# 0xPolygonZero/proof-protocol-decoder

Measured on AMD Instinct MI355X. Metric: txn-proofs/sec (whole node), 256-txn synthetic block, higher is better.
Workload: dtype u64 (Goldilocks field)

## Files before the change

__graft_entry__.py:

```python
import os
import subprocess
import sys

ROOT = os.path.dirname(os.path.abspath(__file__))
if ROOT not in sys.path:
    sys.path.insert(0, ROOT)


def build():
    csrc = os.path.join(ROOT, "proof_protocol_decoder_amd", "csrc")
    subprocess.run(["make", "-C", csrc, "-j8"], check=True)
    subprocess.run(["make", "-C", os.path.join(ROOT, "oracle"), "liboracle.so"], check=True)
    tools = os.path.join(ROOT, "tools")
    subprocess.run(["/opt/rocm/bin/hipcc", "--offload-arch=gfx950", "-O3", "-std=c++17", "-Wno-unused-value", "-o",
                    os.path.join(tools, "microbench"), os.path.join(tools, "microbench.hip")], check=True)
    subprocess.run(["/opt/rocm/bin/hipcc", "--offload-arch=gfx950", "-O2", "-Wno-unused-value", "-o",
                    os.path.join(tools, "wait_probe"), os.path.join(tools, "wait_probe.hip")], check=True)
    subprocess.run(["/opt/rocm/bin/hipcc", "--offload-arch=gfx950", "-O3", "-Wno-unused-value", "-o",
                    os.path.join(tools, "issue_rate"), os.path.join(tools, "issue_rate.hip")], check=True)
    subprocess.run(["/opt/rocm/bin/hipcc", "--offload-arch=gfx950", "-O3", "-Wno-unused-value", "-o",
                    os.path.join(tools, "mfma_probe"), os.path.join(tools, "mfma_probe.hip")], check=True)
    subprocess.run(["/opt/rocm/bin/hipcc", "--offload-arch=gfx950", "-O3", "-std=c++17", "-Wno-unused-value", "-I", csrc,
                    "-mllvm", "-amdgpu-mfma-vgpr-form=1", "-o", os.path.join(tools, "perm_latency"),
                    os.path.join(tools, "perm_latency.hip")], check=True)
    import proof_protocol_decoder_amd as pkg
    pkg.lib()
    return None


def smoke():
    import numpy as np
    import torch
    assert torch.cuda.is_available(), "smoke() needs a GPU"
    import proof_protocol_decoder_amd as pkg
    from proof_protocol_decoder_amd import proof_gen as pg
    from oracle import pyoracle
    sys.path.insert(0, os.path.join(ROOT, "tests"))
    from pg_common import LOG_N, SMALL_PLONK as SMALL, WIDTH, ir_words
    pkg.lib()
    b = pg.ProverStateBuilder()
    for t, name in enumerate(pg.TABLES):
        getattr(b, "set_%s_circuit_size" % name)(range(SMALL["table_log_lo"][t], SMALL["table_log_hi"][t]))
    b.set(**{k: v for k, v in SMALL.items() if not k.startswith("table_")}, n_workers=1, arena_bytes=256 << 20)
    st = b.build()
    try:
        t0 = pg.generate_txn_proof(st, pg.TxnProofGenIR(7, 0, 100, 121, (1, 2, 3, 4), 0x5EED0001, LOG_N, WIDTH))
        t1 = pg.generate_txn_proof(st, pg.TxnProofGenIR(7, 1, 121, 150, t0.p_vals.state_root_after, 0x5EED0002,
                                                        LOG_N, WIDTH))
        agg = pg.generate_agg_proof(st, t0, t1)
        blk = pg.generate_block_proof(st, None, agg)
        pg.VerifierState.from_prover_state(st).verify(blk)
        pyoracle.build()
        ost = pyoracle.PgState(**SMALL)
        want = ost.txn(ir_words(7, 0, 0x5EED0001))
        got = np.frombuffer(t0.intern, dtype=np.uint64)
        assert got.shape == want.shape and (got == want).all(), "txn proof differs from the oracle"
        assert ost.verify(np.frombuffer(blk.intern, dtype=np.uint64)) == 0, "oracle verifier rejected the block proof"
    finally:
        st.close()
    print("smoke ok: txn proof == oracle (%d bytes), block proof verified by both verifiers" % len(t0.intern))
    return None


if __name__ == "__main__":
    build()
    if len(sys.argv) > 1 and sys.argv[1] == "smoke":
        smoke()
```

proof_protocol_decoder_amd/csrc/mx_arith.cuh:

```cuda
#pragma once
#include "gl.hpp"

namespace mxa {

typedef int v4i __attribute__((ext_vector_type(4)));

template <int N>
__device__ __forceinline__ void reduce_rows(const uint64_t (&L)[N], const uint64_t (&H)[N], uint64_t (&out)[N]) {
  uint32_t l0[N], l1[N], h0[N], h1[N];
  uint64_t T[N];
  gl::cc::mask c1[N], b[N];
#pragma unroll
  for (int i = 0; i < N; i++) {
    T[i] = L[i]; h0[i] = (uint32_t)H[i]; h1[i] = (uint32_t)(H[i] >> 32);
  }
  gl::cc::mad_eps_cv(T, h1);
#pragma unroll
  for (int i = 0; i < N; i++) { l0[i] = (uint32_t)T[i]; l1[i] = (uint32_t)(T[i] >> 32); }
  gl::cc::add_co(l1, c1, h0);
  gl::cc::subb0_co(l0, b, c1);
#pragma unroll
  for (int i = 0; i < N; i++) c1[i] &= ~b[i];
  gl::cc::addc0_cv(l1, c1);
#pragma unroll
  for (int i = 0; i < N; i++) out[i] = gl::cc::mk64(l0[i], l1[i]);
}


__device__ __forceinline__ uint64_t planes(const v4i& d) {
  const uint32_t e = (uint32_t)d[0] + ((uint32_t)d[1] << 8), f = (uint32_t)d[2] + ((uint32_t)d[3] << 8);
  uint64_t r;
  asm("v_mad_u64_u32 %0, vcc, %1, %2, %3" : "=v"(r) : "v"(f), "s"(65536u), "v"((uint64_t)e) : "vcc");
  return r;
}

}
```

proof_protocol_decoder_amd/csrc/poseidon_mx.cuh:

```cuda
#pragma once
#include "poseidon.cuh"
#include "poseidon_group.hpp"

namespace poseidon {
namespace mx {

using mxa::v4i;

constexpr int CIN_PER_ROUND = 4 * 24;
constexpr int CIN_WORDS = 30 * CIN_PER_ROUND;

__device__ __forceinline__ uint32_t mds_entry(uint32_t i, uint32_t k) {
  constexpr uint32_t C[12] = {17, 15, 41, 16, 2, 28, 13, 13, 39, 18, 34, 20};
  const uint32_t d = (k + 12 - i) % 12;
  uint32_t v = 0;
#pragma unroll
  for (int j = 0; j < 12; j++) v = d == (uint32_t)j ? C[j] : v;
  return v + ((i | k) == 0 ? 8u : 0u);
}

struct CinTable {
  uint32_t v[CIN_WORDS];
};
constexpr CinTable make_cin_table() {
  constexpr uint64_t rc[360] = {
#include "poseidon_rc.inc"
  };
  CinTable t{};
  for (int i = 0; i < CIN_WORDS; i++) {
    const int rnd = i / CIN_PER_ROUND, rem = i % CIN_PER_ROUND, ib = rem / 24, idx = rem % 24;
    const int g = idx >> 3, h = (idx >> 2) & 1, reg = idx & 3, wo = ib + 4 * g;
    uint32_t v = 128u * (256u + (wo == 0 ? 8u : 0u));
    if (rnd < 29) v += (uint32_t)(rc[(rnd + 1) * 12 + wo] >> (8 * (4 * h + reg))) & 0xFFu;
    t.v[i] = v;
  }
  return t;
}
static __device__ const CinTable CIN_TABLE __attribute__((aligned(16))) = make_cin_table();

__device__ __forceinline__ void build_cin(uint32_t* __restrict__ cin) {
  const uint4* src = (const uint4*)CIN_TABLE.v;
  uint4* dst = (uint4*)cin;
  for (uint32_t i = threadIdx.x; i < (uint32_t)CIN_WORDS / 4; i += blockDim.x) dst[i] = src[i];
}

struct Ctx {
  v4i A[3];
  uint32_t kb;
  const uint32_t* cin;
};
__device__ __forceinline__ Ctx make_ctx(const uint32_t* cin_lds) {
  Ctx c;
  const uint32_t lane = threadIdx.x & 63, r = lane & 15;
  c.kb = lane >> 4;
#pragma unroll
  for (int g = 0; g < 3; g++) {
#pragma unroll
    for (int a = 0; a < 3; a++) c.A[g][a] = (int)(mds_entry((r >> 2) + 4 * g, c.kb + 4 * a) << (8 * (r & 3)));
    c.A[g][3] = 0;
  }
  c.cin = cin_lds + c.kb * 24;
  return c;
}

using mxa::planes;

template <int NS>
__device__ __forceinline__ void mds(uint64_t (&e)[NS][3], const Ctx& c, int rnd) {
  const v4i* cr = (const v4i*)(c.cin + rnd * CIN_PER_ROUND);
  v4i cin[6];
#pragma unroll
  for (int t = 0; t < 6; t++) cin[t] = cr[t];
#pragma unroll
  for (int m = 0; m < NS; m++) {
    v4i blo, bhi;
#pragma unroll
    for (int a = 0; a < 3; a++) {
      blo[a] = (int)((uint32_t)e[m][a] ^ 0x80808080u);
      bhi[a] = (int)((uint32_t)(e[m][a] >> 32) ^ 0x80808080u);
    }
    blo[3] = 0;
    bhi[3] = 0;
    uint64_t L[3], H[3];
#pragma unroll
    for (int g = 0; g < 3; g++) {
      const v4i dl = __builtin_amdgcn_mfma_i32_16x16x64_i8(c.A[g], blo, cin[2 * g], 0, 0, 0);
      const v4i dh = __builtin_amdgcn_mfma_i32_16x16x64_i8(c.A[g], bhi, cin[2 * g + 1], 0, 0, 0);
      L[g] = planes(dl);
      H[g] = planes(dh);
    }
    reduce_rows<3>(L, H, e[m]);
  }
}

template <int NS>
__device__ __forceinline__ void sbox_word0(uint64_t (&e)[NS][3], const Ctx& c) {
  if constexpr (NS == 4) {
    uint32_t l0 = (uint32_t)e[0][0], l1 = (uint32_t)e[1][0], l2 = (uint32_t)e[2][0], l3 = (uint32_t)e[3][0];
    uint32_t h0 = (uint32_t)(e[0][0] >> 32), h1 = (uint32_t)(e[1][0] >> 32), h2 = (uint32_t)(e[2][0] >> 32),
             h3 = (uint32_t)(e[3][0] >> 32);
    asm("s_nop 1\n\t"
        "v_permlane16_swap_b32 %0, %1\n\tv_permlane16_swap_b32 %2, %3\n\t"
        "v_permlane16_swap_b32 %4, %5\n\tv_permlane16_swap_b32 %6, %7\n\t"
        "s_nop 0\n\t"
        "v_permlane32_swap_b32 %0, %2\n\tv_permlane32_swap_b32 %4, %6\n\ts_nop 1"
        : "+v"(l0), "+v"(l1), "+v"(l2), "+v"(l3), "+v"(h0), "+v"(h1), "+v"(h2), "+v"(h3));
    const uint64_t y = sbox(gl::cc::mk64(l0, h0));
    l0 = (uint32_t)y;
    h0 = (uint32_t)(y >> 32);
    asm("s_nop 1\n\t"
        "v_permlane32_swap_b32 %0, %2\n\tv_permlane32_swap_b32 %4, %6\n\t"
        "s_nop 1\n\t"
        "v_permlane16_swap_b32 %0, %1\n\tv_permlane16_swap_b32 %2, %3\n\t"
        "v_permlane16_swap_b32 %4, %5\n\tv_permlane16_swap_b32 %6, %7\n\ts_nop 1"
        : "+v"(l0), "+v"(l1), "+v"(l2), "+v"(l3), "+v"(h0), "+v"(h1), "+v"(h2), "+v"(h3));
    e[0][0] = gl::cc::mk64(l0, h0);
    e[1][0] = gl::cc::mk64(l1, h1);
    e[2][0] = gl::cc::mk64(l2, h2);
    e[3][0] = gl::cc::mk64(l3, h3);
  } else if constexpr (NS == 2) {
    uint32_t l0 = (uint32_t)e[0][0], l1 = (uint32_t)e[1][0], h0 = (uint32_t)(e[0][0] >> 32), h1 = (uint32_t)(e[1][0] >> 32);
    asm("s_nop 1\n\tv_permlane16_swap_b32 %0, %1\n\tv_permlane16_swap_b32 %2, %3\n\ts_nop 1"
        : "+v"(l0), "+v"(l1), "+v"(h0), "+v"(h1));
    const uint64_t y = sbox(gl::cc::mk64(l0, h0));
    const bool word0 = c.kb < 2;
    l0 = word0 ? (uint32_t)y : l0;
    h0 = word0 ? (uint32_t)(y >> 32) : h0;
    asm("s_nop 1\n\tv_permlane16_swap_b32 %0, %1\n\tv_permlane16_swap_b32 %2, %3\n\ts_nop 1"
        : "+v"(l0), "+v"(l1), "+v"(h0), "+v"(h1));
    e[0][0] = gl::cc::mk64(l0, h0);
    e[1][0] = gl::cc::mk64(l1, h1);
  } else {
    static_assert(NS == 1, "1, 2 or 4 sets per wave");
    const uint64_t y = sbox(e[0][0]);
    e[0][0] = c.kb == 0 ? y : e[0][0];
  }
}

template <int NS>
__device__ __forceinline__ void sbox_full(uint64_t (&e)[NS][3]) {
#pragma unroll
  for (int m = 0; m < NS; m++) {
    sbox_n<3>(e[m]);
    __builtin_amdgcn_sched_barrier(0);
  }
}

namespace grp {
constexpr int K = 8;
constexpr poseidon::group::Layout LAY = poseidon::group::layout(K);
constexpr int SHORT_K = 6;
constexpr int OPS_WORDS = LAY.n_ops * 256;
constexpr int C_WORDS = poseidon::group::CFORM_WORDS + poseidon::group::CMAIN_WORDS;
constexpr int MDS_A_WORDS = 3 * 256;
template <int NG> constexpr int TABLE_WORDS = OPS_WORDS + NG * C_WORDS + MDS_A_WORDS;
template <int NG> constexpr int IMAGE_WORDS = TABLE_WORDS<NG> + (NG == 3 ? 18 * 256 : 0);

template <int NG>
__device__ __forceinline__ void load_tables(uint32_t* __restrict__ lds, const uint32_t* __restrict__ glob) {
  const uint4* src = (const uint4*)glob;
  uint4* dst = (uint4*)lds;
  for (uint32_t i = threadIdx.x; i < (uint32_t)TABLE_WORDS<NG> / 4; i += blockDim.x) dst[i] = src[i];
}

template <int F>
__device__ __forceinline__ void gather(uint32_t (&l)[4], uint32_t (&h)[4]) {
  if constexpr ((F & 1) == 0)
    asm("s_nop 1\n\t"
        "v_permlane16_swap_b32 %0, %1\n\tv_permlane16_swap_b32 %2, %3\n\t"
        "v_permlane16_swap_b32 %4, %5\n\tv_permlane16_swap_b32 %6, %7\n\t"
        "s_nop 0\n\t"
        "v_permlane32_swap_b32 %0, %2\n\tv_permlane32_swap_b32 %4, %6\n\ts_nop 1"
        : "+v"(l[0]), "+v"(l[1]), "+v"(l[2]), "+v"(l[3]), "+v"(h[0]), "+v"(h[1]), "+v"(h[2]), "+v"(h[3]));
  else
    asm("s_nop 1\n\t"
        "v_permlane16_swap_b32 %0, %1\n\tv_permlane16_swap_b32 %2, %3\n\t"
        "v_permlane16_swap_b32 %4, %5\n\tv_permlane16_swap_b32 %6, %7\n\t"
        "s_nop 0\n\t"
        "v_permlane32_swap_b32 %1, %3\n\tv_permlane32_swap_b32 %5, %7\n\ts_nop 1"
        : "+v"(l[0]), "+v"(l[1]), "+v"(l[2]), "+v"(l[3]), "+v"(h[0]), "+v"(h[1]), "+v"(h[2]), "+v"(h[3]));
}
template <int F>
__device__ __forceinline__ void scatter(uint32_t (&l)[4], uint32_t (&h)[4]) {
  if constexpr ((F & 1) == 0)
    asm("s_nop 1\n\t"
        "v_permlane32_swap_b32 %0, %2\n\tv_permlane32_swap_b32 %4, %6\n\t"
        "s_nop 1\n\t"
        "v_permlane16_swap_b32 %0, %1\n\tv_permlane16_swap_b32 %2, %3\n\t"
        "v_permlane16_swap_b32 %4, %5\n\tv_permlane16_swap_b32 %6, %7\n\ts_nop 1"
        : "+v"(l[0]), "+v"(l[1]), "+v"(l[2]), "+v"(l[3]), "+v"(h[0]), "+v"(h[1]), "+v"(h[2]), "+v"(h[3]));
  else
    asm("s_nop 1\n\t"
        "v_permlane32_swap_b32 %1, %3\n\tv_permlane32_swap_b32 %5, %7\n\t"
        "s_nop 1\n\t"
        "v_permlane16_swap_b32 %0, %1\n\tv_permlane16_swap_b32 %2, %3\n\t"
        "v_permlane16_swap_b32 %4, %5\n\tv_permlane16_swap_b32 %6, %7\n\ts_nop 1"
        : "+v"(l[0]), "+v"(l[1]), "+v"(l[2]), "+v"(l[3]), "+v"(h[0]), "+v"(h[1]), "+v"(h[2]), "+v"(h[3]));
}

struct State {
  v4i blo[4], bhi[4], bsig[4];
  v4i acc[4][2];
};

template <int J>
__device__ __forceinline__ void step(State& s, uint64_t (&e)[4][3], const v4i* ops, const int* cform, uint32_t lane,
                                     bool full = true) {
  constexpr int P = J / 4, F = J % 4;
  const uint32_t kb = lane >> 4;
  if constexpr (F == 0) {
    constexpr int nw = LAY.w_per_half[P];
#pragma unroll
    for (int half = 0; half < 2; half++) {
      const v4i c0 = ((const v4i*)(cform + (P * 2 + half) * 16))[kb];
      const v4i a_lo = ops[(LAY.w_base[P] + half * nw) * 64 + lane], a_hi = ops[(LAY.w_base[P] + half * nw + 1) * 64 + lane];
#pragma unroll
      for (int m = 0; m < 4; m++) {
        s.acc[m][half] = __builtin_amdgcn_mfma_i32_16x16x64_i8(a_lo, s.blo[m], c0, 0, 0, 0);
        s.acc[m][half] = __builtin_amdgcn_mfma_i32_16x16x64_i8(a_hi, s.bhi[m], s.acc[m][half], 0, 0, 0);
      }
      if constexpr (P > 0) {
        const v4i a_sg = ops[(LAY.w_base[P] + half * nw + 2) * 64 + lane];
#pragma unroll
        for (int m = 0; m < 4; m++) s.acc[m][half] = __builtin_amdgcn_mfma_i32_16x16x64_i8(a_sg, s.bsig[m], s.acc[m][half], 0, 0, 0);
      }
    }
  }
  uint32_t l[4], h[4];
  if constexpr (J == 0) {
#pragma unroll
    for (int m = 0; m < 4; m++) { l[m] = (uint32_t)e[m][0]; h[m] = (uint32_t)(e[m][0] >> 32); }
  } else {
    uint64_t L[4], H[4], x[4];
#pragma unroll
    for (int m = 0; m < 4; m++) { L[m] = planes(s.acc[m][0]); H[m] = planes(s.acc[m][1]); }
    reduce_rows<4>(L, H, x);
#pragma unroll
    for (int m = 0; m < 4; m++) { l[m] = (uint32_t)x[m]; h[m] = (uint32_t)(x[m] >> 32); }
  }
  gather<F>(l, h);
  const uint64_t y = sbox(gl::cc::mk64(l[F], h[F])) ^ 0x8080808080808080ULL;
  l[F] = (uint32_t)y;
  h[F] = (uint32_t)(y >> 32);
  scatter<F>(l, h);
#pragma unroll
  for (int m = 0; m < 4; m++) {
    s.bsig[m][2 * (J / 4)] = __builtin_amdgcn_update_dpp(s.bsig[m][2 * (J / 4)], (int)l[m], 0xE4, 1 << F, 0xF, false);
    s.bsig[m][2 * (J / 4) + 1] = __builtin_amdgcn_update_dpp(s.bsig[m][2 * (J / 4) + 1], (int)h[m], 0xE4, 1 << F, 0xF, false);
  }
  if constexpr (J >= LAY.d_first[P] && J < LAY.d_first[P] + LAY.d_count[P]) {
    if (J == SHORT_K - 1 && !full) return;
#pragma unroll
    for (int half = 0; half < 2; half++) {
      const v4i a = ops[(LAY.d_base[P] + 2 * (J - LAY.d_first[P]) + half) * 64 + lane];
#pragma unroll
      for (int m = 0; m < 4; m++) s.acc[m][half] = __builtin_amdgcn_mfma_i32_16x16x64_i8(a, s.bsig[m], s.acc[m][half], 0, 0, 0);
    }
  }
}

template <int NG>
__device__ __forceinline__ void partial_group(uint64_t (&e)[4][3], const uint32_t* tab, const uint32_t* __restrict__ gtab, int grp) {
  const uint32_t lane = threadIdx.x & 63, kb = lane >> 4;
  const bool full = NG == 2 || grp < 2;
  const v4i* ops = (const v4i*)tab;
  const int* cform = (const int*)(tab + OPS_WORDS + grp * C_WORDS);
  const int* cmain = cform + poseidon::group::CFORM_WORDS;
  State s;
#pragma unroll
  for (int m = 0; m < 4; m++) {
#pragma unroll
    for (int a = 0; a < 3; a++) {
      s.blo[m][a] = (int)((uint32_t)e[m][a] ^ 0x80808080u);
      s.bhi[m][a] = (int)((uint32_t)(e[m][a] >> 32) ^ 0x80808080u);
    }
    s.blo[m][3] = 0;
    s.bhi[m][3] = 0;
    s.bsig[m] = v4i{0, 0, 0, 0};
  }
  step<0>(s, e, ops, cform, lane);
  step<1>(s, e, ops, cform, lane);
  step<2>(s, e, ops, cform, lane);
  step<3>(s, e, ops, cform, lane);
  step<4>(s, e, ops, cform, lane);
  step<5>(s, e, ops, cform, lane, full);
  if (full) {
    step<6>(s, e, ops, cform, lane);
    step<7>(s, e, ops, cform, lane);
  }
  const v4i* lops = ops + LAY.main_base * 64 + lane;
  const v4i* gops = (const v4i*)(gtab + TABLE_WORDS<NG>) + lane;
#pragma unroll
  for (int g = 0; g < 3; g++) {
    v4i d[4][2], A[2][3];
    if (full) {
#pragma unroll
      for (int h = 0; h < 2; h++)
#pragma unroll
        for (int c = 0; c < 3; c++) A[h][c] = lops[((g * 2 + h) * 3 + c) * 64];
    } else {
#pragma unroll
      for (int h = 0; h < 2; h++)
#pragma unroll
        for (int c = 0; c < 3; c++) A[h][c] = gops[((g * 2 + h) * 3 + c) * 64];
    }
#pragma unroll
    for (int h = 0; h < 2; h++) {
      const v4i c0 = ((const v4i*)(cmain + (g * 2 + h) * 16))[kb];
#pragma unroll
      for (int m = 0; m < 4; m++) {
        d[m][h] = __builtin_amdgcn_mfma_i32_16x16x64_i8(A[h][0], s.blo[m], c0, 0, 0, 0);
        d[m][h] = __builtin_amdgcn_mfma_i32_16x16x64_i8(A[h][1], s.bhi[m], d[m][h], 0, 0, 0);
        d[m][h] = __builtin_amdgcn_mfma_i32_16x16x64_i8(A[h][2], s.bsig[m], d[m][h], 0, 0, 0);
      }
    }
    uint64_t L[4], H[4], x[4];
#pragma unroll
    for (int m = 0; m < 4; m++) { L[m] = planes(d[m][0]); H[m] = planes(d[m][1]); }
    reduce_rows<4>(L, H, x);
#pragma unroll
    for (int m = 0; m < 4; m++) e[m][g] = x[m];
  }
}
}

template <int NG> constexpr int CIN_GROUPED_ROUNDS = NG == 3 ? 8 : 14;
template <int NG> constexpr int CIN_GROUPED_WORDS = CIN_GROUPED_ROUNDS<NG> * CIN_PER_ROUND;
template <int NG> __device__ __forceinline__ int cin_slot(int rnd) { return rnd < 4 ? rnd : rnd - (30 - CIN_GROUPED_ROUNDS<NG>); }
template <int NG>
__device__ __forceinline__ void build_cin_grouped(uint32_t* __restrict__ cin) {
  const uint4* src = (const uint4*)CIN_TABLE.v;
  uint4* dst = (uint4*)cin;
  for (uint32_t i = threadIdx.x; i < (uint32_t)CIN_GROUPED_WORDS<NG> / 4; i += blockDim.x)
    dst[i] = src[i < 4 * CIN_PER_ROUND / 4 ? i : i + (30 - CIN_GROUPED_ROUNDS<NG>) * CIN_PER_ROUND / 4];
}

template <int NG>
__device__ __forceinline__ void mds4_lds(uint64_t (&e)[4][3], const Ctx& c, int rnd, const uint32_t* tab) {
  const v4i* cr = (const v4i*)(c.cin + cin_slot<NG>(rnd) * CIN_PER_ROUND);
  const v4i* am = (const v4i*)(tab + grp::OPS_WORDS + NG * grp::C_WORDS) + (threadIdx.x & 63);
#pragma unroll
  for (int m = 0; m < 4; m++) {
    v4i blo, bhi;
#pragma unroll
    for (int a = 0; a < 3; a++) {
      blo[a] = (int)((uint32_t)e[m][a] ^ 0x80808080u);
      bhi[a] = (int)((uint32_t)(e[m][a] >> 32) ^ 0x80808080u);
    }
    blo[3] = 0;
    bhi[3] = 0;
    uint64_t L[3], H[3];
#pragma unroll
    for (int g = 0; g < 3; g++) {
      const v4i A = am[g * 64];
      const v4i dl = __builtin_amdgcn_mfma_i32_16x16x64_i8(A, blo, cr[2 * g], 0, 0, 0);
      const v4i dh = __builtin_amdgcn_mfma_i32_16x16x64_i8(A, bhi, cr[2 * g + 1], 0, 0, 0);
      L[g] = planes(dl);
      H[g] = planes(dh);
    }
    reduce_rows<3>(L, H, e[m]);
  }
}

template <int NG>
__device__ __forceinline__ void permute_grouped(uint64_t (&e)[4][3], const Ctx& c, const uint32_t* tab,
                                                const uint32_t* __restrict__ gtab) {
#pragma unroll
  for (int a = 0; a < 3; a++) {
    const uint64_t k = RC[c.kb + 4 * a];
#pragma unroll
    for (int m = 0; m < 4; m++) e[m][a] = gl::add(e[m][a], k);
  }
  int rnd = 0;
#pragma unroll 1
  for (int k = 0; k < 4; k++, rnd++) {
    sbox_full<4>(e);
    mds4_lds<NG>(e, c, rnd, tab);
  }
#pragma unroll 1
  for (int g = 0; g < NG; g++) grp::partial_group<NG>(e, tab, gtab, g);
  rnd = NG == 3 ? 26 : 20;
  if constexpr (NG == 2) {
#pragma unroll 1
    for (; rnd < 26; rnd++) {
      sbox_word0<4>(e, c);
      mds4_lds<NG>(e, c, rnd, tab);
    }
  }
#pragma unroll 1
  for (int k = 0; k < 4; k++, rnd++) {
    sbox_full<4>(e);
    mds4_lds<NG>(e, c, rnd, tab);
  }
}

template <int NS>
__device__ __forceinline__ void permute(uint64_t (&e)[NS][3], const Ctx& c) {
#pragma unroll
  for (int a = 0; a < 3; a++) {
    const uint64_t k = RC[c.kb + 4 * a];
#pragma unroll
    for (int m = 0; m < NS; m++) e[m][a] = gl::add(e[m][a], k);
  }
  int rnd = 0;
#pragma unroll 1
  for (int k = 0; k < 4; k++, rnd++) {
    sbox_full<NS>(e);
    mds<NS>(e, c, rnd);
  }
#pragma unroll 1
  for (int k = 0; k < 22; k++, rnd++) {
    sbox_word0<NS>(e, c);
    mds<NS>(e, c, rnd);
  }
#pragma unroll 1
  for (int k = 0; k < 4; k++, rnd++) {
    sbox_full<NS>(e);
    mds<NS>(e, c, rnd);
  }
}

}
}
```

Measured before the change: 33.55.

## Replace permlane gather/scatter in grouped Poseidon partial rounds with rotated operand addressing

```diff
diff --git a/__graft_entry__.py b/__graft_entry__.py
--- a/__graft_entry__.py
+++ b/__graft_entry__.py
@@ -23,6 +23,10 @@
     subprocess.run(["/opt/rocm/bin/hipcc", "--offload-arch=gfx950", "-O3", "-std=c++17", "-Wno-unused-value", "-I", csrc,
                     "-mllvm", "-amdgpu-mfma-vgpr-form=1", "-o", os.path.join(tools, "perm_latency"),
                     os.path.join(tools, "perm_latency.hip")], check=True)
+    for out, flags in (("mfma_coexec_probe", ["-mllvm", "-amdgpu-mfma-vgpr-form=1"]),
+                       ("mfma_coexec_probe_agpr", ['-DMFMA_FORM="AGPRs"'])):
+        subprocess.run(["/opt/rocm/bin/hipcc", "--offload-arch=gfx950", "-O3", "-std=c++17", "-Wno-unused-value", "-I", csrc]
+                       + flags + ["-o", os.path.join(tools, out), os.path.join(tools, "mfma_coexec_probe.hip")], check=True)
     import proof_protocol_decoder_amd as pkg
     pkg.lib()
     return None
diff --git a/proof_protocol_decoder_amd/csrc/mx_arith.cuh b/proof_protocol_decoder_amd/csrc/mx_arith.cuh
--- a/proof_protocol_decoder_amd/csrc/mx_arith.cuh
+++ b/proof_protocol_decoder_amd/csrc/mx_arith.cuh
@@ -26,6 +26,14 @@
   for (int i = 0; i < N; i++) out[i] = gl::cc::mk64(l0[i], l1[i]);
 }
 
+__device__ __forceinline__ uint64_t reduce_row(uint64_t L, uint64_t H) {
+  uint64_t T;
+  asm("v_mad_u64_u32 %0, vcc, %1, -1, %2" : "=v"(T) : "v"((uint32_t)(H >> 32)), "v"(L) : "vcc");
+  gl::cc::mask c1, b, unused;
+  const uint32_t l1 = gl::cc::add_co((uint32_t)(T >> 32), (uint32_t)H, c1);
+  const uint32_t l0 = gl::cc::subb0_co((uint32_t)T, c1, b);
+  return gl::cc::mk64(l0, gl::cc::addc0_co(l1, c1 & ~b, unused));
+}
 
 __device__ __forceinline__ uint64_t planes(const v4i& d) {
   const uint32_t e = (uint32_t)d[0] + ((uint32_t)d[1] << 8), f = (uint32_t)d[2] + ((uint32_t)d[3] << 8);
diff --git a/proof_protocol_decoder_amd/csrc/poseidon_mx.cuh b/proof_protocol_decoder_amd/csrc/poseidon_mx.cuh
--- a/proof_protocol_decoder_amd/csrc/poseidon_mx.cuh
+++ b/proof_protocol_decoder_amd/csrc/poseidon_mx.cuh
@@ -163,66 +163,83 @@
   for (uint32_t i = threadIdx.x; i < (uint32_t)TABLE_WORDS<NG> / 4; i += blockDim.x) dst[i] = src[i];
 }
 
-template <int F>
-__device__ __forceinline__ void gather(uint32_t (&l)[4], uint32_t (&h)[4]) {
-  if constexpr ((F & 1) == 0)
-    asm("s_nop 1\n\t"
-        "v_permlane16_swap_b32 %0, %1\n\tv_permlane16_swap_b32 %2, %3\n\t"
-        "v_permlane16_swap_b32 %4, %5\n\tv_permlane16_swap_b32 %6, %7\n\t"
-        "s_nop 0\n\t"
-        "v_permlane32_swap_b32 %0, %2\n\tv_permlane32_swap_b32 %4, %6\n\ts_nop 1"
-        : "+v"(l[0]), "+v"(l[1]), "+v"(l[2]), "+v"(l[3]), "+v"(h[0]), "+v"(h[1]), "+v"(h[2]), "+v"(h[3]));
-  else
-    asm("s_nop 1\n\t"
-        "v_permlane16_swap_b32 %0, %1\n\tv_permlane16_swap_b32 %2, %3\n\t"
-        "v_permlane16_swap_b32 %4, %5\n\tv_permlane16_swap_b32 %6, %7\n\t"
-        "s_nop 0\n\t"
-        "v_permlane32_swap_b32 %1, %3\n\tv_permlane32_swap_b32 %5, %7\n\ts_nop 1"
-        : "+v"(l[0]), "+v"(l[1]), "+v"(l[2]), "+v"(l[3]), "+v"(h[0]), "+v"(h[1]), "+v"(h[2]), "+v"(h[3]));
-}
-template <int F>
-__device__ __forceinline__ void scatter(uint32_t (&l)[4], uint32_t (&h)[4]) {
-  if constexpr ((F & 1) == 0)
-    asm("s_nop 1\n\t"
-        "v_permlane32_swap_b32 %0, %2\n\tv_permlane32_swap_b32 %4, %6\n\t"
-        "s_nop 1\n\t"
-        "v_permlane16_swap_b32 %0, %1\n\tv_permlane16_swap_b32 %2, %3\n\t"
-        "v_permlane16_swap_b32 %4, %5\n\tv_permlane16_swap_b32 %6, %7\n\ts_nop 1"
-        : "+v"(l[0]), "+v"(l[1]), "+v"(l[2]), "+v"(l[3]), "+v"(h[0]), "+v"(h[1]), "+v"(h[2]), "+v"(h[3]));
-  else
-    asm("s_nop 1\n\t"
-        "v_permlane32_swap_b32 %1, %3\n\tv_permlane32_swap_b32 %5, %7\n\t"
-        "s_nop 1\n\t"
-        "v_permlane16_swap_b32 %0, %1\n\tv_permlane16_swap_b32 %2, %3\n\t"
-        "v_permlane16_swap_b32 %4, %5\n\tv_permlane16_swap_b32 %6, %7\n\ts_nop 1"
-        : "+v"(l[0]), "+v"(l[1]), "+v"(l[2]), "+v"(l[3]), "+v"(h[0]), "+v"(h[1]), "+v"(h[2]), "+v"(h[3]));
+__device__ __forceinline__ void gather0(uint32_t (&l)[4], uint32_t (&h)[4]) {
+  asm("s_nop 1\n\t"
+      "v_permlane16_swap_b32 %0, %1\n\tv_permlane16_swap_b32 %2, %3\n\t"
+      "v_permlane16_swap_b32 %4, %5\n\tv_permlane16_swap_b32 %6, %7\n\t"
+      "s_nop 0\n\t"
+      "v_permlane32_swap_b32 %0, %2\n\tv_permlane32_swap_b32 %4, %6\n\ts_nop 1"
+      : "+v"(l[0]), "+v"(l[1]), "+v"(l[2]), "+v"(l[3]), "+v"(h[0]), "+v"(h[1]), "+v"(h[2]), "+v"(h[3]));
+}
+
+template <bool ROWS, bool KBS>
+__device__ __forceinline__ uint32_t rot_lane(uint32_t lane, int m) {
+  const uint32_t r = ROWS ? ((lane - 4u * (uint32_t)m) & 15u) : (lane & 15u);
+  const uint32_t kb = KBS ? (((lane >> 4) - (uint32_t)m) & 3u) : (lane >> 4);
+  return r | kb << 4;
+}
+
+struct Lanes {
+  uint32_t w[4], d[4], s[4];
+};
+__device__ __forceinline__ Lanes lanes_of(uint32_t lane) {
+  Lanes o;
+#pragma unroll
+  for (int m = 0; m < 4; m++) {
+    o.w[m] = rot_lane<true, false>(lane, m) * 16;
+    o.d[m] = rot_lane<true, true>(lane, m) * 16;
+    o.s[m] = rot_lane<false, true>(lane, m) * 16;
+  }
+  return o;
+}
+__device__ __forceinline__ void renew(Lanes& o) {
+  asm volatile("" : "+v"(o.w[0]), "+v"(o.w[1]), "+v"(o.w[2]), "+v"(o.w[3]), "+v"(o.d[1]), "+v"(o.d[2]), "+v"(o.d[3]),
+               "+v"(o.s[1]), "+v"(o.s[2]), "+v"(o.s[3]));
+  o.d[0] = o.s[0] = o.w[0];
+}
+
+__device__ __forceinline__ v4i at(const v4i* image, uint32_t off) {
+  return *(__attribute__((address_space(3))) const v4i*)((__attribute__((address_space(3))) const char*)image + off);
+}
+__device__ __forceinline__ v4i at_global(const v4i* image, uint32_t off) {
+  return *(__attribute__((address_space(1))) const v4i*)((__attribute__((address_space(1))) const char*)image + off);
+}
+
+template <int ROW, int SLOT>
+__device__ __forceinline__ void put_sigma(v4i& b, uint64_t y) {
+  b[SLOT] = __builtin_amdgcn_update_dpp(b[SLOT], (int)(uint32_t)y, 0xE4, 1 << ROW, 0xF, false);
+  b[SLOT + 1] = __builtin_amdgcn_update_dpp(b[SLOT + 1], (int)(uint32_t)(y >> 32), 0xE4, 1 << ROW, 0xF, false);
 }
 
 struct State {
   v4i blo[4], bhi[4], bsig[4];
   v4i acc[4][2];
 };
+__device__ __forceinline__ void init_state(State& s) {
+#pragma unroll
+  for (int m = 0; m < 4; m++) {
+    s.blo[m] = v4i{0, 0, 0, 0};
+    s.bhi[m] = v4i{0, 0, 0, 0};
+    s.bsig[m] = v4i{0, 0, 0, 0};
+  }
+}
 
 template <int J>
-__device__ __forceinline__ void step(State& s, uint64_t (&e)[4][3], const v4i* ops, const int* cform, uint32_t lane,
-                                     bool full = true) {
+__device__ __forceinline__ void step(State& s, uint64_t (&e)[4][3], const v4i* ops, const int* cform, const Lanes& o,
+                                     uint32_t kb, bool full = true) {
   constexpr int P = J / 4, F = J % 4;
-  const uint32_t kb = lane >> 4;
   if constexpr (F == 0) {
     constexpr int nw = LAY.w_per_half[P];
 #pragma unroll
     for (int half = 0; half < 2; half++) {
-      const v4i c0 = ((const v4i*)(cform + (P * 2 + half) * 16))[kb];
-      const v4i a_lo = ops[(LAY.w_base[P] + half * nw) * 64 + lane], a_hi = ops[(LAY.w_base[P] + half * nw + 1) * 64 + lane];
+      const v4i* cf = (const v4i*)(cform + (P * 2 + half) * 16);
+      const v4i* w = ops + (LAY.w_base[P] + half * nw) * 64;
 #pragma unroll
       for (int m = 0; m < 4; m++) {
-        s.acc[m][half] = __builtin_amdgcn_mfma_i32_16x16x64_i8(a_lo, s.blo[m], c0, 0, 0, 0);
-        s.acc[m][half] = __builtin_amdgcn_mfma_i32_16x16x64_i8(a_hi, s.bhi[m], s.acc[m][half], 0, 0, 0);
-      }
-      if constexpr (P > 0) {
-        const v4i a_sg = ops[(LAY.w_base[P] + half * nw + 2) * 64 + lane];
-#pragma unroll
-        for (int m = 0; m < 4; m++) s.acc[m][half] = __builtin_amdgcn_mfma_i32_16x16x64_i8(a_sg, s.bsig[m], s.acc[m][half], 0, 0, 0);
+        s.acc[m][half] = __builtin_amdgcn_mfma_i32_16x16x64_i8(at(w, o.w[m]), s.blo[m], cf[(kb - m) & 3], 0, 0, 0);
+        s.acc[m][half] = __builtin_amdgcn_mfma_i32_16x16x64_i8(at(w + 64, o.w[m]), s.bhi[m], s.acc[m][half], 0, 0, 0);
+        if constexpr (P > 0)
+          s.acc[m][half] = __builtin_amdgcn_mfma_i32_16x16x64_i8(at(w + 128, o.d[m]), s.bsig[m], s.acc[m][half], 0, 0, 0);
       }
     }
   }
@@ -230,43 +247,48 @@
   if constexpr (J == 0) {
 #pragma unroll
     for (int m = 0; m < 4; m++) { l[m] = (uint32_t)e[m][0]; h[m] = (uint32_t)(e[m][0] >> 32); }
+    gather0(l, h);
   } else {
-    uint64_t L[4], H[4], x[4];
-#pragma unroll
-    for (int m = 0; m < 4; m++) { L[m] = planes(s.acc[m][0]); H[m] = planes(s.acc[m][1]); }
-    reduce_rows<4>(L, H, x);
-#pragma unroll
-    for (int m = 0; m < 4; m++) { l[m] = (uint32_t)x[m]; h[m] = (uint32_t)(x[m] >> 32); }
-  }
-  gather<F>(l, h);
-  const uint64_t y = sbox(gl::cc::mk64(l[F], h[F])) ^ 0x8080808080808080ULL;
-  l[F] = (uint32_t)y;
-  h[F] = (uint32_t)(y >> 32);
-  scatter<F>(l, h);
-#pragma unroll
-  for (int m = 0; m < 4; m++) {
-    s.bsig[m][2 * (J / 4)] = __builtin_amdgcn_update_dpp(s.bsig[m][2 * (J / 4)], (int)l[m], 0xE4, 1 << F, 0xF, false);
-    s.bsig[m][2 * (J / 4) + 1] = __builtin_amdgcn_update_dpp(s.bsig[m][2 * (J / 4) + 1], (int)h[m], 0xE4, 1 << F, 0xF, false);
-  }
+    v4i dl = s.acc[(4 - F) & 3][0], dh = s.acc[(4 - F) & 3][1];
+#pragma unroll
+    for (int g = 1; g < 4; g++) {
+      const bool here = kb == (uint32_t)g;
+#pragma unroll
+      for (int q = 0; q < 4; q++) {
+        dl[q] = here ? s.acc[(g - F + 4) & 3][0][q] : dl[q];
+        dh[q] = here ? s.acc[(g - F + 4) & 3][1][q] : dh[q];
+      }
+    }
+    const uint64_t x = mxa::reduce_row(planes(dl), planes(dh));
+    l[0] = (uint32_t)x;
+    h[0] = (uint32_t)(x >> 32);
+  }
+  const uint64_t y = sbox(gl::cc::mk64(l[0], h[0])) ^ 0x8080808080808080ULL;
+  put_sigma<(F + 0) & 3, 2 * P>(s.bsig[0], y);
+  put_sigma<(F + 1) & 3, 2 * P>(s.bsig[1], y);
+  put_sigma<(F + 2) & 3, 2 * P>(s.bsig[2], y);
+  put_sigma<(F + 3) & 3, 2 * P>(s.bsig[3], y);
   if constexpr (J >= LAY.d_first[P] && J < LAY.d_first[P] + LAY.d_count[P]) {
     if (J == SHORT_K - 1 && !full) return;
 #pragma unroll
     for (int half = 0; half < 2; half++) {
-      const v4i a = ops[(LAY.d_base[P] + 2 * (J - LAY.d_first[P]) + half) * 64 + lane];
-#pragma unroll
-      for (int m = 0; m < 4; m++) s.acc[m][half] = __builtin_amdgcn_mfma_i32_16x16x64_i8(a, s.bsig[m], s.acc[m][half], 0, 0, 0);
+      const v4i* a = ops + (LAY.d_base[P] + 2 * (J - LAY.d_first[P]) + half) * 64;
+#pragma unroll
+      for (int m = 0; m < 4; m++)
+        s.acc[m][half] = __builtin_amdgcn_mfma_i32_16x16x64_i8(at(a, o.d[m]), s.bsig[m], s.acc[m][half], 0, 0, 0);
     }
   }
 }
 
 template <int NG>
-__device__ __forceinline__ void partial_group(uint64_t (&e)[4][3], const uint32_t* tab, const uint32_t* __restrict__ gtab, int grp) {
+__device__ __forceinline__ void partial_group(State& s, Lanes& o, uint64_t (&e)[4][3], const uint32_t* tab,
+                                              const uint32_t* __restrict__ gtab, int grp) {
   const uint32_t lane = threadIdx.x & 63, kb = lane >> 4;
   const bool full = NG == 2 || grp < 2;
   const v4i* ops = (const v4i*)tab;
   const int* cform = (const int*)(tab + OPS_WORDS + grp * C_WORDS);
   const int* cmain = cform + poseidon::group::CFORM_WORDS;
-  State s;
+  renew(o);
 #pragma unroll
   for (int m = 0; m < 4; m++) {
 #pragma unroll
@@ -274,44 +296,43 @@
       s.blo[m][a] = (int)((uint32_t)e[m][a] ^ 0x80808080u);
       s.bhi[m][a] = (int)((uint32_t)(e[m][a] >> 32) ^ 0x80808080u);
     }
-    s.blo[m][3] = 0;
-    s.bhi[m][3] = 0;
-    s.bsig[m] = v4i{0, 0, 0, 0};
-  }
-  step<0>(s, e, ops, cform, lane);
-  step<1>(s, e, ops, cform, lane);
-  step<2>(s, e, ops, cform, lane);
-  step<3>(s, e, ops, cform, lane);
-  step<4>(s, e, ops, cform, lane);
-  step<5>(s, e, ops, cform, lane, full);
+  }
+  step<0>(s, e, ops, cform, o, kb);
+  step<1>(s, e, ops, cform, o, kb);
+  step<2>(s, e, ops, cform, o, kb);
+  step<3>(s, e, ops, cform, o, kb);
+  step<4>(s, e, ops, cform, o, kb);
+  step<5>(s, e, ops, cform, o, kb, full);
   if (full) {
-    step<6>(s, e, ops, cform, lane);
-    step<7>(s, e, ops, cform, lane);
-  }
-  const v4i* lops = ops + LAY.main_base * 64 + lane;
-  const v4i* gops = (const v4i*)(gtab + TABLE_WORDS<NG>) + lane;
+    step<6>(s, e, ops, cform, o, kb);
+    step<7>(s, e, ops, cform, o, kb);
+  }
+  const v4i* lops = ops + LAY.main_base * 64;
+  const v4i* gops = (const v4i*)(gtab + TABLE_WORDS<NG>);
 #pragma unroll
   for (int g = 0; g < 3; g++) {
-    v4i d[4][2], A[2][3];
-    if (full) {
-#pragma unroll
-      for (int h = 0; h < 2; h++)
-#pragma unroll
-        for (int c = 0; c < 3; c++) A[h][c] = lops[((g * 2 + h) * 3 + c) * 64];
-    } else {
-#pragma unroll
-      for (int h = 0; h < 2; h++)
-#pragma unroll
-        for (int c = 0; c < 3; c++) A[h][c] = gops[((g * 2 + h) * 3 + c) * 64];
-    }
+    v4i d[4][2];
 #pragma unroll
     for (int h = 0; h < 2; h++) {
+      const int t = (g * 2 + h) * 3 * 64;
+      v4i a_lo, a_hi, a_sg[4];
+      if (full) {
+        a_lo = at(lops + t, o.s[0]);
+        a_hi = at(lops + t + 64, o.s[0]);
+#pragma unroll
+        for (int m = 0; m < 4; m++) a_sg[m] = at(lops + t + 128, o.s[m]);
+      } else {
+        a_lo = at_global(gops + t, o.s[0]);
+        a_hi = at_global(gops + t + 64, o.s[0]);
+#pragma unroll
+        for (int m = 0; m < 4; m++) a_sg[m] = at_global(gops + t + 128, o.s[m]);
+      }
       const v4i c0 = ((const v4i*)(cmain + (g * 2 + h) * 16))[kb];
 #pragma unroll
       for (int m = 0; m < 4; m++) {
-        d[m][h] = __builtin_amdgcn_mfma_i32_16x16x64_i8(A[h][0], s.blo[m], c0, 0, 0, 0);
-        d[m][h] = __builtin_amdgcn_mfma_i32_16x16x64_i8(A[h][1], s.bhi[m], d[m][h], 0, 0, 0);
-        d[m][h] = __builtin_amdgcn_mfma_i32_16x16x64_i8(A[h][2], s.bsig[m], d[m][h], 0, 0, 0);
+        d[m][h] = __builtin_amdgcn_mfma_i32_16x16x64_i8(a_lo, s.blo[m], c0, 0, 0, 0);
+        d[m][h] = __builtin_amdgcn_mfma_i32_16x16x64_i8(a_hi, s.bhi[m], d[m][h], 0, 0, 0);
+        d[m][h] = __builtin_amdgcn_mfma_i32_16x16x64_i8(a_sg[m], s.bsig[m], d[m][h], 0, 0, 0);
       }
     }
     uint64_t L[4], H[4], x[4];
@@ -377,8 +398,11 @@
     sbox_full<4>(e);
     mds4_lds<NG>(e, c, rnd, tab);
   }
-#pragma unroll 1
-  for (int g = 0; g < NG; g++) grp::partial_group<NG>(e, tab, gtab, g);
+  grp::State s;
+  grp::init_state(s);
+  grp::Lanes o = grp::lanes_of(threadIdx.x & 63);
+#pragma unroll 1
+  for (int g = 0; g < NG; g++) grp::partial_group<NG>(s, o, e, tab, gtab, g);
   rnd = NG == 3 ? 26 : 20;
   if constexpr (NG == 2) {
 #pragma unroll 1
```

New measurement: 34.25 (median of 6 runs). 1.02x the previous value.
